# lilijiangg/AutoDiffusion

Hardware: AMD Instinct MI355X
Metric: images/sec (node), ADM-G ImageNet-64 4-step DDIM (higher is better)
Workload: dtype bf16

## Files before the change

autodiffusion_amd/csrc/adm_attention.hip:

```cpp
#include <stdlib.h>

#include <type_traits>

#include "adm_attn_common.h"

namespace {

constexpr int KT = 64;
constexpr int QW = 32;
constexpr int QB = 128;
constexpr int PADE = 16;

#ifdef ADM_ATTN_TIMING
__device__ unsigned long long adm_attn_timing_buf[8 * 65536];
#define ATT_T0() unsigned long long tph[8] = {0, 0, 0, 0, 0, 0, 0, 0}; unsigned long long tlast = __builtin_amdgcn_s_memtime()
#define ATT_T(k) do { const unsigned long long tn_ = __builtin_amdgcn_s_memtime(); tph[k] += tn_ - tlast; tlast = tn_; } while (0)
#define ATT_TEND() do { if (threadIdx.x == 0) { const unsigned b_ = blockIdx.x + gridDim.x * blockIdx.y; if (b_ < 65536) for (int i_ = 0; i_ < 8; ++i_) adm_attn_timing_buf[b_ * 8 + i_] = tph[i_]; } } while (0)
#else
#define ATT_T0() do {} while (0)
#define ATT_T(k) do {} while (0)
#define ATT_TEND() do {} while (0)
#endif

struct AttnK {
  const uint16_t* qkv; uint16_t* out; float* lse;
  const uint16_t* kv;
  int T, heads, C3, C;
  int Tk, kv_rows, Ckv;
  int q_off, k_off, v_off, head_stride, kv_head_stride;
  float scale_log2;
};

template <int D>
__global__ void __launch_bounds__(256, D <= 64 ? 3 : 2)
attn_kernel(const AttnK p) {
  constexpr int KS = D / 32;
  constexpr bool R16 = (D % 32) == 16;
  static_assert(D % 16 == 0 && KS >= 1, "head width must be a multiple of 16, at least 32");
  constexpr int DT = D / 16;
  constexpr float MOVE_THR = 8.0f;
  constexpr bool DMA = D == 64;
  constexpr int KROW = DMA ? D : D + (((D / 2) % 16 == 8) ? 0 : PADE);
  __shared__ __attribute__((aligned(16))) uint16_t Ks[2][KT * KROW];
  __shared__ __attribute__((aligned(16))) uint16_t Vs[2][KT * KROW];

  const int tid = threadIdx.x, lane = tid & 63, wave = tid >> 6;
  const int lc = lane & 15, lq = lane >> 4;
  int bx, by;
  adm_xcd_block(bx, by);
  const int n = by / p.heads, hd = by % p.heads;
  const int qbase = bx * QB + wave * QW;
  const uint16_t* base = p.qkv + (long long)n * p.T * p.C3;
  const int qcol = p.q_off + hd * p.head_stride, kcol = p.k_off + hd * p.kv_head_stride,
            vcol = p.v_off + hd * p.kv_head_stride;
  const __amdgpu_buffer_rsrc_t rsk = __builtin_amdgcn_make_buffer_rsrc((void*)(p.kv + (long long)n * p.kv_rows * p.Ckv), 0,
                                                                       p.Tk * p.Ckv * 2, 0x00020000);

  const __amdgpu_buffer_rsrc_t rs = __builtin_amdgcn_make_buffer_rsrc((void*)base, 0, p.T * p.C3 * 2, 0x00020000);
  adm_h8 qf[2][KS];
#pragma unroll
  for (int qt = 0; qt < 2; ++qt) {
    const int q = qbase + qt * 16 + lc;
#pragma unroll
    for (int ks = 0; ks < KS; ++ks) {
      const adm_u32x4 v = __builtin_amdgcn_raw_buffer_load_b128(rs, (q * p.C3 + qcol + ks * 32 + lq * 8) * 2, 0, 0);
      qf[qt][ks] = __builtin_bit_cast(adm_h8, v);
    }
  }
  adm_s16x4 qf16[2] = {};
  if constexpr (R16) {
#pragma unroll
    for (int qt = 0; qt < 2; ++qt) {
      const int q = qbase + qt * 16 + lc;
      const adm_u32x2 v = __builtin_amdgcn_raw_buffer_load_b64(rs, (q * p.C3 + qcol + KS * 32 + lq * 4) * 2, 0, 0);
      qf16[qt] = __builtin_bit_cast(adm_s16x4, v);
    }
  }

  f32x4 oacc[DT][2], lacc[2], cin[2];
#pragma unroll
  for (int qt = 0; qt < 2; ++qt) {
#pragma unroll
    for (int dt = 0; dt < DT; ++dt) oacc[dt][qt] = f32x4{0.f, 0.f, 0.f, 0.f};
    lacc[qt] = f32x4{0.f, 0.f, 0.f, 0.f};
    cin[qt] = f32x4{0.f, 0.f, 0.f, 0.f};
  }
  float m_run[2] = {0.f, 0.f};
  typedef __attribute__((ext_vector_type(8))) short s16x8;
  const adm_h8 ones = __builtin_bit_cast(adm_h8, s16x8{ADM_ONE16, ADM_ONE16, ADM_ONE16, ADM_ONE16, ADM_ONE16, ADM_ONE16, ADM_ONE16, ADM_ONE16});
  const float thr_raw = MOVE_THR / p.scale_log2;

  const int ntiles = (p.Tk + KT - 1) / KT;
  ATT_T0();
  AdmTileRegs<KT, D, 256> kr, vr;
  typedef __attribute__((ext_vector_type(4))) unsigned int u32x4s;
  const unsigned long long kvbase = (unsigned long long)(p.kv + (long long)n * p.kv_rows * p.Ckv);
  const u32x4s rsk_s = {(unsigned)__builtin_amdgcn_readfirstlane((int)(unsigned)kvbase),
                        (unsigned)__builtin_amdgcn_readfirstlane((int)(unsigned)(kvbase >> 32)) & 0xffffu,
                        (unsigned)__builtin_amdgcn_readfirstlane(p.Tk * p.Ckv * 2), 0x00020000u};
  const unsigned lds_k = (unsigned)(uintptr_t)(__attribute__((address_space(3))) uint16_t*)&Ks[0][0];
  const unsigned lds_v = (unsigned)(uintptr_t)(__attribute__((address_space(3))) uint16_t*)&Vs[0][0];
  const int wave_u = __builtin_amdgcn_readfirstlane(wave);
  auto dma_tile = [&](int kt0) {
    const unsigned slot = (unsigned)(kt0 & 1) * (KT * KROW * 2);
#pragma unroll
    for (int j = 0; j < 2; ++j) {
      const int piece = wave_u * 2 + j;
      const int row = kt0 * KT + piece * 8 + (lane >> 3);
      const int gseg = (lane & 7) ^ (lane >> 3);
      const unsigned voff_k = (unsigned)(row * p.Ckv + kcol + gseg * 8) * 2u, voff_v = (unsigned)(row * p.Ckv + vcol + gseg * 8) * 2u;
      const unsigned dst_k = lds_k + slot + piece * 1024, dst_v = lds_v + slot + piece * 1024;
      unsigned keep;
      asm volatile("s_mov_b32 %0, m0\n\ts_mov_b32 m0, %3\n\ts_nop 0\n\tbuffer_load_dwordx4 %1, %2, 0 offen lds\n\ts_mov_b32 m0, %0"
                   : "=&s"(keep) : "v"(voff_k), "s"(rsk_s), "s"(dst_k) : "memory");
      asm volatile("s_mov_b32 %0, m0\n\ts_mov_b32 m0, %3\n\ts_nop 0\n\tbuffer_load_dwordx4 %1, %2, 0 offen lds\n\ts_mov_b32 m0, %0"
                   : "=&s"(keep) : "v"(voff_v), "s"(rsk_s), "s"(dst_v) : "memory");
    }
  };
  if constexpr (DMA) {
    dma_tile(0);
    asm volatile("s_waitcnt vmcnt(0)" ::: "memory");
  } else {
    kr.load_buf(rsk, p.Ckv, kcol, 0, tid);
    vr.load_buf(rsk, p.Ckv, vcol, 0, tid);
    kr.store(Ks[0], KROW, tid);
    vr.store(Vs[0], KROW, tid);
  }
  __syncthreads();

  auto s_phase = [&](int kt0, f32x4 (&st)[4][2]) {
    const uint16_t* Kc = Ks[kt0 & 1];
    constexpr int NSET = R16 ? 4 : 2;
    adm_h8 kfr[NSET][KS];
    adm_s16x4 kfr16[NSET] = {};
    auto kread = [&](int kt) {
      const int slot = kt % NSET;
#pragma unroll
      for (int ks = 0; ks < KS; ++ks)
        kfr[slot][ks] = *reinterpret_cast<const adm_h8*>(
            &Kc[(kt * 16 + lc) * KROW + (DMA ? ((ks * 4 + lq) ^ (lc & 7)) * 8 : ks * 32 + lq * 8)]);
      if constexpr (R16) kfr16[slot] = *reinterpret_cast<const adm_s16x4*>(&Kc[(kt * 16 + lc) * KROW + KS * 32 + lq * 4]);
    };
    __builtin_amdgcn_sched_barrier(0);
    if constexpr (R16) {
#pragma unroll
      for (int kt = 0; kt < 4; ++kt) kread(kt);
    } else {
      kread(0);
    }
#pragma unroll
    for (int kt = 0; kt < 4; ++kt) {
      if (!R16 && kt + 1 < 4) kread(kt + 1);
      __builtin_amdgcn_sched_barrier(0);
#pragma unroll
      for (int qt = 0; qt < 2; ++qt)
        st[kt][qt] = adm_mfma_16x16x32(kfr[kt % NSET][0], qf[qt][0], cin[qt], 0, 0, 0);
#pragma unroll
      for (int ks = 1; ks < KS; ++ks)
#pragma unroll
        for (int qt = 0; qt < 2; ++qt)
          st[kt][qt] = adm_mfma_16x16x32(kfr[kt % NSET][ks], qf[qt][ks], st[kt][qt], 0, 0, 0);
      if constexpr (R16) {
#pragma unroll
        for (int qt = 0; qt < 2; ++qt)
          st[kt][qt] = adm_mfma_16x16x16(kfr16[kt % NSET], qf16[qt], st[kt][qt], 0, 0, 0);
      }
      __builtin_amdgcn_sched_barrier(0);
    }
  };

  auto tile = [&](int kt0, auto rag_, auto first_) {
    constexpr bool RAG = decltype(rag_)::value, FIRST = decltype(first_)::value;
    const int k0 = kt0 * KT;
    const bool next = kt0 + 1 < ntiles;
    if (next) {
      if constexpr (DMA) {
        dma_tile(kt0 + 1);
      } else {
        kr.load_buf(rsk, p.Ckv, kcol, k0 + KT, tid);
        vr.load_buf(rsk, p.Ckv, vcol, k0 + KT, tid);
      }
    }
    ATT_T(0);
    f32x4 st[4][2];
    s_phase(kt0, st);
    ATT_T(1);
    const uint16_t* Vc = Vs[kt0 & 1];
    __builtin_amdgcn_sched_barrier(0);
    adm_h8 vfr[2][2];
    auto vread = [&](int dt, int slot) {
#pragma unroll
      for (int kb = 0; kb < 2; ++kb)
        vfr[slot][kb] = DMA ? adm_tr_frag_swz(Vc, kb * 32, dt * 16, lc, lq) : adm_tr_frag(Vc, KROW, kb * 32, dt * 16, lc, lq);
    };
    vread(0, 0);
    __builtin_amdgcn_sched_barrier(0);
    ATT_T(2);
    if constexpr (RAG) {
#pragma unroll
// ... 288 lines not shown
```

autodiffusion_amd/csrc/adm_attention_bwd.hip:

```cpp
#include "adm_attn_common.h"

namespace {

constexpr int TT = 64;
constexpr int BW = 32;
constexpr int BB = 128;
constexpr int PADE = 16;

struct AttnBwdK {
  const uint16_t* qkv; const uint16_t* out; const uint16_t* dout; const float* lse; const float* delta;
  float* delta_out;
  uint16_t* dqkv;
  int T, heads, C3, C;
  int q_off, k_off, v_off, head_stride;
  float scale_log2, inv_sqrt_d;
};

template <int D>
__global__ void __launch_bounds__(256, 2)
attn_dq_kernel(const AttnBwdK p) {
  constexpr int KS = D / 32, DT = D / 16, KROW = D + PADE;
  __shared__ __attribute__((aligned(16))) uint16_t Ks[2][TT * KROW];
  __shared__ __attribute__((aligned(16))) uint16_t Vs[2][TT * KROW];
  const int tid = threadIdx.x, lane = tid & 63, wave = tid >> 6, lc = lane & 15, lq = lane >> 4;
  int bx, by;
  adm_xcd_block(bx, by);
  const int n = by / p.heads, hd = by % p.heads;
  const int qbase = bx * BB + wave * BW;
  const uint16_t* base = p.qkv + (long long)n * p.T * p.C3;
  const uint16_t* dbase = p.dout + (long long)n * p.T * p.C;
  const int qcol = p.q_off + hd * p.head_stride, kcol = p.k_off + hd * p.head_stride, vcol = p.v_off + hd * p.head_stride;

  const __amdgpu_buffer_rsrc_t rs = __builtin_amdgcn_make_buffer_rsrc((void*)base, 0, p.T * p.C3 * 2, 0x00020000);
  const __amdgpu_buffer_rsrc_t rsg = __builtin_amdgcn_make_buffer_rsrc((void*)dbase, 0, p.T * p.C * 2, 0x00020000);
  const __amdgpu_buffer_rsrc_t rso = __builtin_amdgcn_make_buffer_rsrc((void*)(p.out + (long long)n * p.T * p.C), 0, p.T * p.C * 2, 0x00020000);
  adm_h8 qf[2][KS], gf[2][KS];
  float lse[2], dl[2];
#pragma unroll
  for (int qt = 0; qt < 2; ++qt) {
    const int q = qbase + qt * 16 + lc;
    const bool ok = q < p.T;
    float dsum = 0.f;
#pragma unroll
    for (int ks = 0; ks < KS; ++ks) {
      const adm_u32x4 a = __builtin_amdgcn_raw_buffer_load_b128(rs, (q * p.C3 + qcol + ks * 32 + lq * 8) * 2, 0, 0);
      const adm_u32x4 g = __builtin_amdgcn_raw_buffer_load_b128(rsg, (q * p.C + hd * D + ks * 32 + lq * 8) * 2, 0, 0);
      const adm_u32x4 o = __builtin_amdgcn_raw_buffer_load_b128(rso, (q * p.C + hd * D + ks * 32 + lq * 8) * 2, 0, 0);
      qf[qt][ks] = __builtin_bit_cast(adm_h8, a);
      gf[qt][ks] = __builtin_bit_cast(adm_h8, g);
#pragma unroll
      for (int e = 0; e < 4; ++e) {
        dsum += adm_lo_f32(o[e]) * adm_lo_f32(g[e]);
        dsum += adm_hi_f32(o[e]) * adm_hi_f32(g[e]);
      }
    }
    dsum = adm_quarter_sum(dsum);
    const long long si = ((long long)n * p.heads + hd) * p.T + (ok ? q : 0);
    lse[qt] = ok ? p.lse[si] : 0.f;
    dl[qt] = dsum;
    if (ok && lq == 0) p.delta_out[si] = dsum;
  }
  f32x4 acc[DT][2];
#pragma unroll
  for (int dt = 0; dt < DT; ++dt)
#pragma unroll
    for (int qt = 0; qt < 2; ++qt) acc[dt][qt] = f32x4{0.f, 0.f, 0.f, 0.f};

  AdmTileRegs<TT, D, 256> kr, vr;
  kr.load_buf(rs, p.C3, kcol, 0, tid);
  vr.load_buf(rs, p.C3, vcol, 0, tid);
  kr.store(Ks[0], KROW, tid);
  vr.store(Vs[0], KROW, tid);
  __syncthreads();

  const int ntiles = (p.T + TT - 1) / TT;
  for (int t0 = 0; t0 < ntiles; ++t0) {
    const int k0 = t0 * TT, cur = t0 & 1;
    const bool next = t0 + 1 < ntiles;
    if (next) {
      kr.load_buf(rs, p.C3, kcol, k0 + TT, tid);
      vr.load_buf(rs, p.C3, vcol, k0 + TT, tid);
    }
    const uint16_t* Kc = Ks[cur];
    const uint16_t* Vc = Vs[cur];
    adm_h8 dsf[2][2];
#pragma unroll
    for (int kb = 0; kb < 2; ++kb) {
      f32x4 st[2][2], dp[2][2];
      const f32x4 zero4 = {0.f, 0.f, 0.f, 0.f};
#pragma unroll
      for (int kk = 0; kk < 2; ++kk) {
        const int kt = 2 * kb + kk;
#pragma unroll
        for (int ks = 0; ks < KS; ++ks) {
          const adm_h8 kf = *reinterpret_cast<const adm_h8*>(&Kc[(kt * 16 + lc) * KROW + ks * 32 + lq * 8]);
          const adm_h8 vf = *reinterpret_cast<const adm_h8*>(&Vc[(kt * 16 + lc) * KROW + ks * 32 + lq * 8]);
#pragma unroll
          for (int qt = 0; qt < 2; ++qt) {
            st[kk][qt] = adm_mfma_16x16x32(kf, qf[qt][ks], ks == 0 ? zero4 : st[kk][qt], 0, 0, 0);
            dp[kk][qt] = adm_mfma_16x16x32(vf, gf[qt][ks], ks == 0 ? zero4 : dp[kk][qt], 0, 0, 0);
          }
        }
      }
#pragma unroll
      for (int qt = 0; qt < 2; ++qt) {
        const adm_f32x2 sc2 = {p.scale_log2, p.scale_log2}, nl2 = {-lse[qt], -lse[qt]}, nd2 = {-dl[qt], -dl[qt]};
        float dsv[8];
#pragma unroll
        for (int kk = 0; kk < 2; ++kk)
#pragma unroll
          for (int h = 0; h < 2; ++h) {
            const adm_f32x2 a = __builtin_elementwise_fma(adm_f32x2{st[kk][qt][2 * h], st[kk][qt][2 * h + 1]}, sc2, nl2);
            const adm_f32x2 pr = {__builtin_amdgcn_exp2f(a.x), __builtin_amdgcn_exp2f(a.y)};
            const adm_f32x2 d2 = pr * (adm_f32x2{dp[kk][qt][2 * h], dp[kk][qt][2 * h + 1]} + nd2);
            dsv[kk * 4 + 2 * h] = d2.x;
            dsv[kk * 4 + 2 * h + 1] = d2.y;
          }
        adm_h8 f;
#pragma unroll
        for (int e = 0; e < 8; ++e) f[e] = (adm_elem_t)dsv[e];
        dsf[qt][kb] = f;
      }
    }
#pragma unroll
    for (int dt = 0; dt < DT; ++dt)
#pragma unroll
      for (int kb = 0; kb < 2; ++kb) {
        const adm_h8 kt_f = adm_tr_frag(Kc, KROW, kb * 32, dt * 16, lc, lq);
#pragma unroll
        for (int qt = 0; qt < 2; ++qt)
          acc[dt][qt] = adm_mfma_16x16x32(kt_f, dsf[qt][kb], acc[dt][qt], 0, 0, 0);
      }
    if (next) {
      kr.store(Ks[cur ^ 1], KROW, tid);
      vr.store(Vs[cur ^ 1], KROW, tid);
    }
    __syncthreads();
  }
#pragma unroll
  for (int qt = 0; qt < 2; ++qt) {
    const int q = qbase + qt * 16 + lc;
    if (q >= p.T) continue;
    uint16_t* orow = p.dqkv + ((long long)n * p.T + q) * p.C3 + qcol;
#pragma unroll
    for (int dt = 0; dt < DT; ++dt) {
      const f32x4 o = acc[dt][qt] * p.inv_sqrt_d;
      uint2 pk;
      pk.x = adm_pack2(o[0], o[1]);
      pk.y = adm_pack2(o[2], o[3]);
      *reinterpret_cast<uint2*>(orow + dt * 16 + lq * 4) = pk;
    }
  }
}

template <int D>
__global__ void __launch_bounds__(256, 2)
attn_dkv_kernel(const AttnBwdK p) {
  constexpr int KS = D / 32, DT = D / 16, KROW = D + PADE;
  __shared__ __attribute__((aligned(16))) uint16_t Qs[2][TT * KROW];
  __shared__ __attribute__((aligned(16))) uint16_t Gs[2][TT * KROW];
  __shared__ __attribute__((aligned(16))) float lse_s[2][TT], dl_s[2][TT];
  const int tid = threadIdx.x, lane = tid & 63, wave = tid >> 6, lc = lane & 15, lq = lane >> 4;
  int bx, by;
  adm_xcd_block(bx, by);
  const int n = by / p.heads, hd = by % p.heads;
  const int kbase = bx * BB + wave * BW;
  const uint16_t* base = p.qkv + (long long)n * p.T * p.C3;
  const uint16_t* dbase = p.dout + (long long)n * p.T * p.C;
  const int qcol = p.q_off + hd * p.head_stride, kcol = p.k_off + hd * p.head_stride, vcol = p.v_off + hd * p.head_stride;
  const long long sbase = ((long long)n * p.heads + hd) * p.T;

  const __amdgpu_buffer_rsrc_t rs = __builtin_amdgcn_make_buffer_rsrc((void*)base, 0, p.T * p.C3 * 2, 0x00020000);
  const __amdgpu_buffer_rsrc_t rsg = __builtin_amdgcn_make_buffer_rsrc((void*)dbase, 0, p.T * p.C * 2, 0x00020000);
  adm_h8 kf[2][KS], vf[2][KS];
#pragma unroll
  for (int kt = 0; kt < 2; ++kt) {
    const int key = kbase + kt * 16 + lc;
#pragma unroll
    for (int ks = 0; ks < KS; ++ks) {
      const adm_u32x4 a = __builtin_amdgcn_raw_buffer_load_b128(rs, (key * p.C3 + kcol + ks * 32 + lq * 8) * 2, 0, 0);
      const adm_u32x4 b = __builtin_amdgcn_raw_buffer_load_b128(rs, (key * p.C3 + vcol + ks * 32 + lq * 8) * 2, 0, 0);
      kf[kt][ks] = __builtin_bit_cast(adm_h8, a);
      vf[kt][ks] = __builtin_bit_cast(adm_h8, b);
    }
  }
  f32x4 dv[DT][2], dk[DT][2];
#pragma unroll
  for (int dt = 0; dt < DT; ++dt)
#pragma unroll
    for (int kt = 0; kt < 2; ++kt) { dv[dt][kt] = f32x4{0.f, 0.f, 0.f, 0.f}; dk[dt][kt] = f32x4{0.f, 0.f, 0.f, 0.f}; }

  AdmTileRegs<TT, D, 256> qr, gr;
  float lse_r = 0.f, dl_r = 0.f;
  auto load_rows = [&](int q0) {
    qr.load_buf(rs, p.C3, qcol, q0, tid);
    gr.load_buf(rsg, p.C, hd * D, q0, tid);
    if (tid < TT) {
      const int q = q0 + tid;
      lse_r = q < p.T ? p.lse[sbase + q] : 1e30f;
      dl_r = q < p.T ? p.delta[sbase + q] : 0.f;
    }
  };
  auto store_rows = [&](int buf) {
    qr.store(Qs[buf], KROW, tid);
    gr.store(Gs[buf], KROW, tid);
    if (tid < TT) { lse_s[buf][tid] = lse_r; dl_s[buf][tid] = dl_r; }
  };
  load_rows(0);
  store_rows(0);
  __syncthreads();

  const int ntiles = (p.T + TT - 1) / TT;
  for (int t0 = 0; t0 < ntiles; ++t0) {
    const int q0 = t0 * TT, cur = t0 & 1;
    const bool next = t0 + 1 < ntiles;
    if (next) load_rows(q0 + TT);
    const uint16_t* Qc = Qs[cur];
    const uint16_t* Gc = Gs[cur];
#pragma unroll
    for (int qb = 0; qb < 2; ++qb) {
      adm_h8 pf[2], dsf[2];
#pragma unroll
      for (int kt = 0; kt < 2; ++kt) {
        f32x4 st[2], dp[2];
        const f32x4 zero4 = {0.f, 0.f, 0.f, 0.f};
#pragma unroll
        for (int qq = 0; qq < 2; ++qq) {
          const int qt = 2 * qb + qq;
#pragma unroll
          for (int ks = 0; ks < KS; ++ks) {
            const adm_h8 qa = *reinterpret_cast<const adm_h8*>(&Qc[(qt * 16 + lc) * KROW + ks * 32 + lq * 8]);
            const adm_h8 ga = *reinterpret_cast<const adm_h8*>(&Gc[(qt * 16 + lc) * KROW + ks * 32 + lq * 8]);
            st[qq] = adm_mfma_16x16x32(qa, kf[kt][ks], ks == 0 ? zero4 : st[qq], 0, 0, 0);
            dp[qq] = adm_mfma_16x16x32(ga, vf[kt][ks], ks == 0 ? zero4 : dp[qq], 0, 0, 0);
          }
        }
        adm_h8 f, g;
        const adm_f32x2 sc2 = {p.scale_log2, p.scale_log2};
#pragma unroll
        for (int qq = 0; qq < 2; ++qq) {
          const int ql = (2 * qb + qq) * 16 + lq * 4;
          const float4 l4 = *reinterpret_cast<const float4*>(&lse_s[cur][ql]);
          const float4 d4 = *reinterpret_cast<const float4*>(&dl_s[cur][ql]);
          const adm_f32x2 a0 = __builtin_elementwise_fma(adm_f32x2{st[qq][0], st[qq][1]}, sc2, adm_f32x2{-l4.x, -l4.y});
          const adm_f32x2 a1 = __builtin_elementwise_fma(adm_f32x2{st[qq][2], st[qq][3]}, sc2, adm_f32x2{-l4.z, -l4.w});
          const adm_f32x2 p0 = {__builtin_amdgcn_exp2f(a0.x), __builtin_amdgcn_exp2f(a0.y)};
          const adm_f32x2 p1 = {__builtin_amdgcn_exp2f(a1.x), __builtin_amdgcn_exp2f(a1.y)};
          const adm_f32x2 s0 = p0 * (adm_f32x2{dp[qq][0], dp[qq][1]} - adm_f32x2{d4.x, d4.y});
          const adm_f32x2 s1 = p1 * (adm_f32x2{dp[qq][2], dp[qq][3]} - adm_f32x2{d4.z, d4.w});
          f[qq * 4 + 0] = (adm_elem_t)p0.x; f[qq * 4 + 1] = (adm_elem_t)p0.y; f[qq * 4 + 2] = (adm_elem_t)p1.x; f[qq * 4 + 3] = (adm_elem_t)p1.y;
          g[qq * 4 + 0] = (adm_elem_t)s0.x; g[qq * 4 + 1] = (adm_elem_t)s0.y; g[qq * 4 + 2] = (adm_elem_t)s1.x; g[qq * 4 + 3] = (adm_elem_t)s1.y;
        }
        pf[kt] = f;
        dsf[kt] = g;
      }
#pragma unroll
      for (int dt = 0; dt < DT; ++dt) {
        const adm_h8 gt_f = adm_tr_frag(Gc, KROW, qb * 32, dt * 16, lc, lq);
        const adm_h8 qt_f = adm_tr_frag(Qc, KROW, qb * 32, dt * 16, lc, lq);
#pragma unroll
        for (int kt = 0; kt < 2; ++kt) {
          dv[dt][kt] = adm_mfma_16x16x32(gt_f, pf[kt], dv[dt][kt], 0, 0, 0);
          dk[dt][kt] = adm_mfma_16x16x32(qt_f, dsf[kt], dk[dt][kt], 0, 0, 0);
        }
      }
    }
    if (next) store_rows(cur ^ 1);
    __syncthreads();
  }
#pragma unroll
  for (int kt = 0; kt < 2; ++kt) {
    const int key = kbase + kt * 16 + lc;
    if (key >= p.T) continue;
    uint16_t* orow = p.dqkv + ((long long)n * p.T + key) * p.C3;
#pragma unroll
    for (int dt = 0; dt < DT; ++dt) {
      const f32x4 a = dk[dt][kt] * p.inv_sqrt_d;
      const f32x4 b = dv[dt][kt];
      uint2 pk;
      pk.x = adm_pack2(a[0], a[1]);
      pk.y = adm_pack2(a[2], a[3]);
      *reinterpret_cast<uint2*>(orow + kcol + dt * 16 + lq * 4) = pk;
      pk.x = adm_pack2(b[0], b[1]);
      pk.y = adm_pack2(b[2], b[3]);
      *reinterpret_cast<uint2*>(orow + vcol + dt * 16 + lq * 4) = pk;
    }
  }
}

}

extern "C" int adm_attention_bwd(const adm_bf16* qkv, const adm_bf16* out, const adm_bf16* dout, const float* lse,
                                 float* delta_ws, adm_bf16* dqkv, int n, int t, int heads, int d, int new_order,
                                 void* stream) {
  ADM_REQUIRE(qkv && out && dout && lse && delta_ws && dqkv, ADM_E_ARG, "adm_attention_bwd: null pointer");
  ADM_REQUIRE(n > 0 && t > 0 && heads > 0, ADM_E_ARG, "adm_attention_bwd: bad shape");
  ADM_REQUIRE(d == 32 || d == 64, ADM_E_SHAPE, "adm_attention_bwd: head dim %d unsupported (32, 64)", d);
  ADM_REQUIRE(adm_aligned16(qkv) && adm_aligned16(out) && adm_aligned16(dout) && adm_aligned16(dqkv), ADM_E_ALIGN,
              "adm_attention_bwd: unaligned pointer");
  ADM_REQUIRE((long long)n * heads < 65536, ADM_E_SHAPE, "adm_attention_bwd: n*heads exceeds grid.y");
  AttnBwdK k{};
  k.qkv = qkv; k.out = out; k.dout = dout; k.lse = lse; k.delta = delta_ws; k.delta_out = delta_ws; k.dqkv = dqkv;
  k.T = t; k.heads = heads; k.C = heads * d; k.C3 = 3 * k.C;
  if (new_order) { k.q_off = 0; k.k_off = k.C; k.v_off = 2 * k.C; k.head_stride = d; }
  else           { k.q_off = 0; k.k_off = d;   k.v_off = 2 * d;   k.head_stride = 3 * d; }
  k.inv_sqrt_d = 1.0f / sqrtf((float)d);
  k.scale_log2 = 1.4426950408889634f * k.inv_sqrt_d;
  hipStream_t s = (hipStream_t)stream;
  dim3 grid((t + BB - 1) / BB, n * heads);
  if (d == 32) {
    hipLaunchKernelGGL((attn_dq_kernel<32>), grid, dim3(256), 0, s, k);
    hipLaunchKernelGGL((attn_dkv_kernel<32>), grid, dim3(256), 0, s, k);
  } else {
    hipLaunchKernelGGL((attn_dq_kernel<64>), grid, dim3(256), 0, s, k);
    hipLaunchKernelGGL((attn_dkv_kernel<64>), grid, dim3(256), 0, s, k);
  }
  return adm_check_launch("adm_attention_bwd");
}
```

autodiffusion_amd/csrc/adm_attn_common.h:

```cpp
#pragma once
#include "adm_common.h"

typedef __attribute__((ext_vector_type(4))) short adm_s16x4;
typedef __attribute__((ext_vector_type(4))) unsigned int adm_u32x4;
typedef __attribute__((ext_vector_type(2))) float adm_f32x2;

__device__ __forceinline__ void adm_xcd_block(int& bx, int& by) {
  const unsigned nx = gridDim.x, total = gridDim.x * gridDim.y;
  const unsigned lin = blockIdx.x + nx * blockIdx.y;
  const unsigned share = total >> 3, rem = total & 7, xcd = lin & 7;
  const unsigned logical = xcd * share + min(xcd, rem) + (lin >> 3);
  bx = (int)(logical % nx);
  by = (int)(logical / nx);
}

__device__ __forceinline__ adm_h8 adm_tr_frag(const uint16_t* tile, int row_stride, int row0, int col0, int lc, int lq) {
  const uint16_t* p0 = tile + (row0 + 4 * lq + (lc >> 2)) * row_stride + col0 + 4 * (lc & 3);
  const adm_s16x4 lo = __builtin_amdgcn_ds_read_tr16_b64_v4i16((__attribute__((address_space(3))) adm_s16x4*)p0);
  const adm_s16x4 hi = __builtin_amdgcn_ds_read_tr16_b64_v4i16(
      (__attribute__((address_space(3))) adm_s16x4*)(p0 + 16 * row_stride));
  typedef __attribute__((ext_vector_type(8))) short s16x8;
  const s16x8 v = {lo[0], lo[1], lo[2], lo[3], hi[0], hi[1], hi[2], hi[3]};
  return __builtin_bit_cast(adm_h8, v);
}

__device__ __forceinline__ adm_h8 adm_tr_frag_swz(const uint16_t* tile, int row0, int col0, int lc, int lq) {
  const int r = 4 * lq + (lc >> 2);
  const int seg = ((col0 >> 3) + ((lc & 3) >> 1)) ^ (r & 7);
  const uint16_t* p0 = tile + (row0 + r) * 64 + seg * 8 + 4 * (lc & 1);
  const adm_s16x4 lo = __builtin_amdgcn_ds_read_tr16_b64_v4i16((__attribute__((address_space(3))) adm_s16x4*)p0);
  const adm_s16x4 hi = __builtin_amdgcn_ds_read_tr16_b64_v4i16((__attribute__((address_space(3))) adm_s16x4*)(p0 + 16 * 64));
  typedef __attribute__((ext_vector_type(8))) short s16x8;
  const s16x8 v = {lo[0], lo[1], lo[2], lo[3], hi[0], hi[1], hi[2], hi[3]};
  return __builtin_bit_cast(adm_h8, v);
}

template <int ROWS, int D, int NT>
struct AdmTileRegs {
  static constexpr int UNITS = ROWS * D / 8;
  static constexpr int PER = (UNITS + NT - 1) / NT;
  uint4 v[PER];
  __device__ __forceinline__ void load(const uint16_t* base, long long row_stride, int col0, int r0, int rmax, int tid) {
#pragma unroll
    for (int i = 0; i < PER; ++i) {
      const int u = tid + i * NT;
      const int r = u / (D / 8), sg = u % (D / 8);
      uint4 x = make_uint4(0, 0, 0, 0);
      if (u < UNITS && r0 + r < rmax) x = *reinterpret_cast<const uint4*>(base + (long long)(r0 + r) * row_stride + col0 + sg * 8);
      v[i] = x;
    }
  }
  __device__ __forceinline__ void load_buf(__amdgpu_buffer_rsrc_t rs, int row_stride, int col0, int r0, int tid) {
#pragma unroll
    for (int i = 0; i < PER; ++i) {
      const int u = tid + i * NT;
      const int r = u / (D / 8), sg = u % (D / 8);
      const unsigned off = u < UNITS ? (unsigned)((r0 + r) * row_stride + col0 + sg * 8) * 2u : 0x80000000u;
      const adm_u32x4 x = __builtin_amdgcn_raw_buffer_load_b128(rs, (int)off, 0, 0);
      v[i] = make_uint4(x[0], x[1], x[2], x[3]);
    }
  }
  __device__ __forceinline__ void store(uint16_t* tile, int krow, int tid) const {
#pragma unroll
    for (int i = 0; i < PER; ++i) {
      const int u = tid + i * NT;
      if (u < UNITS) *reinterpret_cast<uint4*>(&tile[(u / (D / 8)) * krow + (u % (D / 8)) * 8]) = v[i];
    }
  }
};

typedef __attribute__((ext_vector_type(2))) unsigned int adm_u32x2;
__device__ __forceinline__ float adm_quarter_max(float x) {
  adm_u32x2 r = __builtin_amdgcn_permlane16_swap(__float_as_uint(x), __float_as_uint(x), false, false);
  const float m = fmaxf(__uint_as_float(r[0]), __uint_as_float(r[1]));
  r = __builtin_amdgcn_permlane32_swap(__float_as_uint(m), __float_as_uint(m), false, false);
  return fmaxf(__uint_as_float(r[0]), __uint_as_float(r[1]));
}
__device__ __forceinline__ float adm_quarter_sum(float x) {
  adm_u32x2 r = __builtin_amdgcn_permlane16_swap(__float_as_uint(x), __float_as_uint(x), false, false);
  const float m = __uint_as_float(r[0]) + __uint_as_float(r[1]);
  r = __builtin_amdgcn_permlane32_swap(__float_as_uint(m), __float_as_uint(m), false, false);
  return __uint_as_float(r[0]) + __uint_as_float(r[1]);
}
```

Measured before the change: 777.4.

## Use LDS-DMA swizzled tile loads and pipelined fragment reads in attention backward

For head dim 64 and sequence length up to a fixed cap, the dQ and dK/dV attention-backward kernels now stream K/V (or Q/dO) tiles straight into LDS. They use buffer_load...lds DMA into an XOR-swizzled, unpadded layout instead of staging through registers. The inner loops are software-pipelined so the next LDS fragment read is issued while the current MFMAs run, with sched_barriers fencing the phases. The dK/dV kernel preloads all lse/delta values into LDS once, and launch bounds rise to three blocks per CU. The aim is less register pressure and fewer VGPR round trips for tile staging, plus better overlap of LDS reads with MFMA. The cost is a hard sequence-length cap, which also makes the LDS footprint larger, and some shared helpers refactored out of the forward kernel.

```diff
diff --git a/autodiffusion_amd/csrc/adm_attention.hip b/autodiffusion_amd/csrc/adm_attention.hip
--- a/autodiffusion_amd/csrc/adm_attention.hip
+++ b/autodiffusion_amd/csrc/adm_attention.hip
@@ -93,11 +93,7 @@
   const int ntiles = (p.Tk + KT - 1) / KT;
   ATT_T0();
   AdmTileRegs<KT, D, 256> kr, vr;
-  typedef __attribute__((ext_vector_type(4))) unsigned int u32x4s;
-  const unsigned long long kvbase = (unsigned long long)(p.kv + (long long)n * p.kv_rows * p.Ckv);
-  const u32x4s rsk_s = {(unsigned)__builtin_amdgcn_readfirstlane((int)(unsigned)kvbase),
-                        (unsigned)__builtin_amdgcn_readfirstlane((int)(unsigned)(kvbase >> 32)) & 0xffffu,
-                        (unsigned)__builtin_amdgcn_readfirstlane(p.Tk * p.Ckv * 2), 0x00020000u};
+  const adm_rsrc_s rsk_s = adm_dma_rsrc(p.kv + (long long)n * p.kv_rows * p.Ckv, p.Tk, p.Ckv);
   const unsigned lds_k = (unsigned)(uintptr_t)(__attribute__((address_space(3))) uint16_t*)&Ks[0][0];
   const unsigned lds_v = (unsigned)(uintptr_t)(__attribute__((address_space(3))) uint16_t*)&Vs[0][0];
   const int wave_u = __builtin_amdgcn_readfirstlane(wave);
@@ -107,14 +103,11 @@
     for (int j = 0; j < 2; ++j) {
       const int piece = wave_u * 2 + j;
       const int row = kt0 * KT + piece * 8 + (lane >> 3);
-      const int gseg = (lane & 7) ^ (lane >> 3);
+      const int gseg = adm_dma_swz_seg(lane);
       const unsigned voff_k = (unsigned)(row * p.Ckv + kcol + gseg * 8) * 2u, voff_v = (unsigned)(row * p.Ckv + vcol + gseg * 8) * 2u;
       const unsigned dst_k = lds_k + slot + piece * 1024, dst_v = lds_v + slot + piece * 1024;
-      unsigned keep;
-      asm volatile("s_mov_b32 %0, m0\n\ts_mov_b32 m0, %3\n\ts_nop 0\n\tbuffer_load_dwordx4 %1, %2, 0 offen lds\n\ts_mov_b32 m0, %0"
-                   : "=&s"(keep) : "v"(voff_k), "s"(rsk_s), "s"(dst_k) : "memory");
-      asm volatile("s_mov_b32 %0, m0\n\ts_mov_b32 m0, %3\n\ts_nop 0\n\tbuffer_load_dwordx4 %1, %2, 0 offen lds\n\ts_mov_b32 m0, %0"
-                   : "=&s"(keep) : "v"(voff_v), "s"(rsk_s), "s"(dst_v) : "memory");
+      adm_lds_dma_b128(voff_k, rsk_s, dst_k);
+      adm_lds_dma_b128(voff_v, rsk_s, dst_v);
     }
   };
   if constexpr (DMA) {
diff --git a/autodiffusion_amd/csrc/adm_attention_bwd.hip b/autodiffusion_amd/csrc/adm_attention_bwd.hip
--- a/autodiffusion_amd/csrc/adm_attention_bwd.hip
+++ b/autodiffusion_amd/csrc/adm_attention_bwd.hip
@@ -6,6 +6,7 @@
 constexpr int BW = 32;
 constexpr int BB = 128;
 constexpr int PADE = 16;
+constexpr int DMA_MAX_T = 2560;
 
 struct AttnBwdK {
   const uint16_t* qkv; const uint16_t* out; const uint16_t* dout; const float* lse; const float* delta;
@@ -16,10 +17,17 @@
   float scale_log2, inv_sqrt_d;
 };
 
-template <int D>
-__global__ void __launch_bounds__(256, 2)
+__device__ __forceinline__ void adm_landed(adm_h8& x) {
+  adm_u32x4 t = __builtin_bit_cast(adm_u32x4, x);
+  asm volatile("" : "+v"(t));
+  x = __builtin_bit_cast(adm_h8, t);
+}
+
+template <int D, bool DMA>
+__global__ void __launch_bounds__(256, DMA ? 3 : 2)
 attn_dq_kernel(const AttnBwdK p) {
-  constexpr int KS = D / 32, DT = D / 16, KROW = D + PADE;
+  static_assert(!DMA || D == 64, "the LDS-DMA tile layout is 128-byte rows");
+  constexpr int KS = D / 32, DT = D / 16, KROW = DMA ? D : D + PADE;
   __shared__ __attribute__((aligned(16))) uint16_t Ks[2][TT * KROW];
   __shared__ __attribute__((aligned(16))) uint16_t Vs[2][TT * KROW];
   const int tid = threadIdx.x, lane = tid & 63, wave = tid >> 6, lc = lane & 15, lq = lane >> 4;
@@ -66,76 +74,158 @@
 #pragma unroll
     for (int qt = 0; qt < 2; ++qt) acc[dt][qt] = f32x4{0.f, 0.f, 0.f, 0.f};
 
-  AdmTileRegs<TT, D, 256> kr, vr;
-  kr.load_buf(rs, p.C3, kcol, 0, tid);
-  vr.load_buf(rs, p.C3, vcol, 0, tid);
-  kr.store(Ks[0], KROW, tid);
-  vr.store(Vs[0], KROW, tid);
-  __syncthreads();
+  auto ds_frag = [&](const f32x4 (&st)[2][2], const f32x4 (&dp)[2][2], int qt) {
+    const adm_f32x2 sc2 = {p.scale_log2, p.scale_log2}, nl2 = {-lse[qt], -lse[qt]}, nd2 = {-dl[qt], -dl[qt]};
+    float dsv[8];
+#pragma unroll
+    for (int kk = 0; kk < 2; ++kk)
+#pragma unroll
+      for (int h = 0; h < 2; ++h) {
+        const adm_f32x2 a = __builtin_elementwise_fma(adm_f32x2{st[kk][qt][2 * h], st[kk][qt][2 * h + 1]}, sc2, nl2);
+        const adm_f32x2 pr = {__builtin_amdgcn_exp2f(a.x), __builtin_amdgcn_exp2f(a.y)};
+        const adm_f32x2 d2 = pr * (adm_f32x2{dp[kk][qt][2 * h], dp[kk][qt][2 * h + 1]} + nd2);
+        dsv[kk * 4 + 2 * h] = d2.x;
+        dsv[kk * 4 + 2 * h + 1] = d2.y;
+      }
+    adm_h8 f;
+#pragma unroll
+    for (int e = 0; e < 8; ++e) f[e] = (adm_elem_t)dsv[e];
+    return f;
+  };
 
   const int ntiles = (p.T + TT - 1) / TT;
-  for (int t0 = 0; t0 < ntiles; ++t0) {
-    const int k0 = t0 * TT, cur = t0 & 1;
-    const bool next = t0 + 1 < ntiles;
-    if (next) {
-      kr.load_buf(rs, p.C3, kcol, k0 + TT, tid);
-      vr.load_buf(rs, p.C3, vcol, k0 + TT, tid);
-    }
-    const uint16_t* Kc = Ks[cur];
-    const uint16_t* Vc = Vs[cur];
-    adm_h8 dsf[2][2];
-#pragma unroll
-    for (int kb = 0; kb < 2; ++kb) {
-      f32x4 st[2][2], dp[2][2];
-      const f32x4 zero4 = {0.f, 0.f, 0.f, 0.f};
-#pragma unroll
-      for (int kk = 0; kk < 2; ++kk) {
-        const int kt = 2 * kb + kk;
+  if constexpr (DMA) {
+    const adm_rsrc_s rs_s = adm_dma_rsrc(base, p.T, p.C3);
+    const unsigned lds_k = (unsigned)(uintptr_t)(__attribute__((address_space(3))) uint16_t*)&Ks[0][0];
+    const unsigned lds_v = (unsigned)(uintptr_t)(__attribute__((address_space(3))) uint16_t*)&Vs[0][0];
+    const int wave_u = __builtin_amdgcn_readfirstlane(wave);
+    auto dma_tile = [&](int t) {
+      const unsigned slot = (unsigned)(t & 1) * (TT * KROW * 2);
+#pragma unroll
+      for (int j = 0; j < 2; ++j) {
+        const int piece = wave_u * 2 + j;
+        const int row_off = (t * TT + piece * 8 + (lane >> 3)) * p.C3 + adm_dma_swz_seg(lane) * 8;
+        adm_lds_dma_b128((unsigned)(row_off + kcol) * 2u, rs_s, lds_k + slot + piece * 1024);
+        adm_lds_dma_b128((unsigned)(row_off + vcol) * 2u, rs_s, lds_v + slot + piece * 1024);
+      }
+    };
+    dma_tile(0);
+#pragma unroll
+    for (int qt = 0; qt < 2; ++qt)
+#pragma unroll
+      for (int ks = 0; ks < KS; ++ks) { adm_landed(qf[qt][ks]); adm_landed(gf[qt][ks]); }
+    asm volatile("s_waitcnt vmcnt(0)" ::: "memory");
+    __syncthreads();
+    for (int t0 = 0; t0 < ntiles; ++t0) {
+      if (t0 + 1 < ntiles) dma_tile(t0 + 1);
+      const uint16_t* Kc = Ks[t0 & 1];
+      const uint16_t* Vc = Vs[t0 & 1];
+      adm_h8 kfr[2][KS], vfr[2][KS], tfr[2][2];
+      auto sread = [&](int kt) {
 #pragma unroll
         for (int ks = 0; ks < KS; ++ks) {
-          const adm_h8 kf = *reinterpret_cast<const adm_h8*>(&Kc[(kt * 16 + lc) * KROW + ks * 32 + lq * 8]);
-          const adm_h8 vf = *reinterpret_cast<const adm_h8*>(&Vc[(kt * 16 + lc) * KROW + ks * 32 + lq * 8]);
-#pragma unroll
-          for (int qt = 0; qt < 2; ++qt) {
-            st[kk][qt] = adm_mfma_16x16x32(kf, qf[qt][ks], ks == 0 ? zero4 : st[kk][qt], 0, 0, 0);
-            dp[kk][qt] = adm_mfma_16x16x32(vf, gf[qt][ks], ks == 0 ? zero4 : dp[kk][qt], 0, 0, 0);
+          const int off = adm_swz_frag_off(kt * 16 + lc, ks * 4 + lq);
+          kfr[kt & 1][ks] = *reinterpret_cast<const adm_h8*>(&Kc[off]);
+          vfr[kt & 1][ks] = *reinterpret_cast<const adm_h8*>(&Vc[off]);
+        }
+      };
+      auto tread = [&](int dt) {
+#pragma unroll
+        for (int kb = 0; kb < 2; ++kb) tfr[dt & 1][kb] = adm_tr_frag_swz(Kc, kb * 32, dt * 16, lc, lq);
+      };
+      adm_h8 dsf[2][2];
+      __builtin_amdgcn_sched_barrier(0);
+      sread(0);
+#pragma unroll
+      for (int kb = 0; kb < 2; ++kb) {
+        f32x4 st[2][2], dp[2][2];
+        const f32x4 zero4 = {0.f, 0.f, 0.f, 0.f};
+#pragma unroll
+        for (int kk = 0; kk < 2; ++kk) {
+          const int kt = 2 * kb + kk;
+          if (kt + 1 < 4) sread(kt + 1); else tread(0);
+          __builtin_amdgcn_sched_barrier(0);
+#pragma unroll
+          for (int ks = 0; ks < KS; ++ks)
+#pragma unroll
+            for (int qt = 0; qt < 2; ++qt) {
+              st[kk][qt] = adm_mfma_16x16x32(kfr[kt & 1][ks], qf[qt][ks], ks == 0 ? zero4 : st[kk][qt], 0, 0, 0);
+              dp[kk][qt] = adm_mfma_16x16x32(vfr[kt & 1][ks], gf[qt][ks], ks == 0 ? zero4 : dp[kk][qt], 0, 0, 0);
+            }
+          __builtin_amdgcn_sched_barrier(0);
+        }
+#pragma unroll
+        for (int qt = 0; qt < 2; ++qt) dsf[qt][kb] = ds_frag(st, dp, qt);
+      }
+      __builtin_amdgcn_sched_barrier(0);
+#pragma unroll
+      for (int dt = 0; dt < DT; ++dt) {
+        if (dt + 1 < DT) tread(dt + 1);
+        __builtin_amdgcn_sched_barrier(0);
+#pragma unroll
+        for (int kb = 0; kb < 2; ++kb)
+#pragma unroll
+          for (int qt = 0; qt < 2; ++qt)
+            acc[dt][qt] = adm_mfma_16x16x32(tfr[dt & 1][kb], dsf[qt][kb], acc[dt][qt], 0, 0, 0);
+        __builtin_amdgcn_sched_barrier(0);
+      }
+      asm volatile("s_waitcnt vmcnt(0)" ::: "memory");
+      __syncthreads();
+    }
+  } else {
+    AdmTileRegs<TT, D, 256> kr, vr;
+    kr.load_buf(rs, p.C3, kcol, 0, tid);
+    vr.load_buf(rs, p.C3, vcol, 0, tid);
+    kr.store(Ks[0], KROW, tid);
+    vr.store(Vs[0], KROW, tid);
+    __syncthreads();
+
+    for (int t0 = 0; t0 < ntiles; ++t0) {
+      const int k0 = t0 * TT, cur = t0 & 1;
+      const bool next = t0 + 1 < ntiles;
+      if (next) {
+        kr.load_buf(rs, p.C3, kcol, k0 + TT, tid);
+        vr.load_buf(rs, p.C3, vcol, k0 + TT, tid);
+      }
+      const uint16_t* Kc = Ks[cur];
+      const uint16_t* Vc = Vs[cur];
+      adm_h8 dsf[2][2];
+#pragma unroll
+      for (int kb = 0; kb < 2; ++kb) {
+        f32x4 st[2][2], dp[2][2];
+        const f32x4 zero4 = {0.f, 0.f, 0.f, 0.f};
+#pragma unroll
+        for (int kk = 0; kk < 2; ++kk) {
+          const int kt = 2 * kb + kk;
+#pragma unroll
+          for (int ks = 0; ks < KS; ++ks) {
+            const adm_h8 kf = *reinterpret_cast<const adm_h8*>(&Kc[(kt * 16 + lc) * KROW + ks * 32 + lq * 8]);
+            const adm_h8 vf = *reinterpret_cast<const adm_h8*>(&Vc[(kt * 16 + lc) * KROW + ks * 32 + lq * 8]);
+#pragma unroll
+            for (int qt = 0; qt < 2; ++qt) {
+              st[kk][qt] = adm_mfma_16x16x32(kf, qf[qt][ks], ks == 0 ? zero4 : st[kk][qt], 0, 0, 0);
+              dp[kk][qt] = adm_mfma_16x16x32(vf, gf[qt][ks], ks == 0 ? zero4 : dp[kk][qt], 0, 0, 0);
+            }
           }
         }
-      }
-#pragma unroll
-      for (int qt = 0; qt < 2; ++qt) {
-        const adm_f32x2 sc2 = {p.scale_log2, p.scale_log2}, nl2 = {-lse[qt], -lse[qt]}, nd2 = {-dl[qt], -dl[qt]};
-        float dsv[8];
-#pragma unroll
-        for (int kk = 0; kk < 2; ++kk)
-#pragma unroll
-          for (int h = 0; h < 2; ++h) {
-            const adm_f32x2 a = __builtin_elementwise_fma(adm_f32x2{st[kk][qt][2 * h], st[kk][qt][2 * h + 1]}, sc2, nl2);
-            const adm_f32x2 pr = {__builtin_amdgcn_exp2f(a.x), __builtin_amdgcn_exp2f(a.y)};
-            const adm_f32x2 d2 = pr * (adm_f32x2{dp[kk][qt][2 * h], dp[kk][qt][2 * h + 1]} + nd2);
-            dsv[kk * 4 + 2 * h] = d2.x;
-            dsv[kk * 4 + 2 * h + 1] = d2.y;
-          }
-        adm_h8 f;
-#pragma unroll
-        for (int e = 0; e < 8; ++e) f[e] = (adm_elem_t)dsv[e];
-        dsf[qt][kb] = f;
-      }
-    }
-#pragma unroll
-    for (int dt = 0; dt < DT; ++dt)
-#pragma unroll
-      for (int kb = 0; kb < 2; ++kb) {
-        const adm_h8 kt_f = adm_tr_frag(Kc, KROW, kb * 32, dt * 16, lc, lq);
-#pragma unroll
-        for (int qt = 0; qt < 2; ++qt)
-          acc[dt][qt] = adm_mfma_16x16x32(kt_f, dsf[qt][kb], acc[dt][qt], 0, 0, 0);
-      }
-    if (next) {
-      kr.store(Ks[cur ^ 1], KROW, tid);
-      vr.store(Vs[cur ^ 1], KROW, tid);
-    }
-    __syncthreads();
+#pragma unroll
+        for (int qt = 0; qt < 2; ++qt) dsf[qt][kb] = ds_frag(st, dp, qt);
+      }
+#pragma unroll
+      for (int dt = 0; dt < DT; ++dt)
+#pragma unroll
+        for (int kb = 0; kb < 2; ++kb) {
+          const adm_h8 kt_f = adm_tr_frag(Kc, KROW, kb * 32, dt * 16, lc, lq);
+#pragma unroll
+          for (int qt = 0; qt < 2; ++qt)
+            acc[dt][qt] = adm_mfma_16x16x32(kt_f, dsf[qt][kb], acc[dt][qt], 0, 0, 0);
+        }
+      if (next) {
+        kr.store(Ks[cur ^ 1], KROW, tid);
+        vr.store(Vs[cur ^ 1], KROW, tid);
+      }
+      __syncthreads();
+    }
   }
 #pragma unroll
   for (int qt = 0; qt < 2; ++qt) {
@@ -153,13 +243,13 @@
   }
 }
 
-template <int D>
-__global__ void __launch_bounds__(256, 2)
+template <int D, bool DMA>
+__global__ void __launch_bounds__(256, DMA ? 3 : 2)
 attn_dkv_kernel(const AttnBwdK p) {
-  constexpr int KS = D / 32, DT = D / 16, KROW = D + PADE;
+  static_assert(!DMA || D == 64, "the LDS-DMA tile layout is 128-byte rows");
+  constexpr int KS = D / 32, DT = D / 16, KROW = DMA ? D : D + PADE;
   __shared__ __attribute__((aligned(16))) uint16_t Qs[2][TT * KROW];
   __shared__ __attribute__((aligned(16))) uint16_t Gs[2][TT * KROW];
-  __shared__ __attribute__((aligned(16))) float lse_s[2][TT], dl_s[2][TT];
   const int tid = threadIdx.x, lane = tid & 63, wave = tid >> 6, lc = lane & 15, lq = lane >> 4;
   int bx, by;
   adm_xcd_block(bx, by);
@@ -190,83 +280,166 @@
 #pragma unroll
     for (int kt = 0; kt < 2; ++kt) { dv[dt][kt] = f32x4{0.f, 0.f, 0.f, 0.f}; dk[dt][kt] = f32x4{0.f, 0.f, 0.f, 0.f}; }
 
-  AdmTileRegs<TT, D, 256> qr, gr;
-  float lse_r = 0.f, dl_r = 0.f;
-  auto load_rows = [&](int q0) {
-    qr.load_buf(rs, p.C3, qcol, q0, tid);
-    gr.load_buf(rsg, p.C, hd * D, q0, tid);
-    if (tid < TT) {
-      const int q = q0 + tid;
-      lse_r = q < p.T ? p.lse[sbase + q] : 1e30f;
-      dl_r = q < p.T ? p.delta[sbase + q] : 0.f;
-    }
+  auto p_ds_frags = [&](const f32x4 (&st)[2], const f32x4 (&dp)[2], const float* l, const float* d, adm_h8& pf, adm_h8& dsf) {
+    adm_h8 f, g;
+    const adm_f32x2 sc2 = {p.scale_log2, p.scale_log2};
+#pragma unroll
+    for (int qq = 0; qq < 2; ++qq) {
+      const float4 l4 = *reinterpret_cast<const float4*>(l + qq * 16);
+      const float4 d4 = *reinterpret_cast<const float4*>(d + qq * 16);
+      const adm_f32x2 a0 = __builtin_elementwise_fma(adm_f32x2{st[qq][0], st[qq][1]}, sc2, adm_f32x2{-l4.x, -l4.y});
+      const adm_f32x2 a1 = __builtin_elementwise_fma(adm_f32x2{st[qq][2], st[qq][3]}, sc2, adm_f32x2{-l4.z, -l4.w});
+      const adm_f32x2 p0 = {__builtin_amdgcn_exp2f(a0.x), __builtin_amdgcn_exp2f(a0.y)};
+      const adm_f32x2 p1 = {__builtin_amdgcn_exp2f(a1.x), __builtin_amdgcn_exp2f(a1.y)};
+      const adm_f32x2 s0 = p0 * (adm_f32x2{dp[qq][0], dp[qq][1]} - adm_f32x2{d4.x, d4.y});
+      const adm_f32x2 s1 = p1 * (adm_f32x2{dp[qq][2], dp[qq][3]} - adm_f32x2{d4.z, d4.w});
+      f[qq * 4 + 0] = (adm_elem_t)p0.x; f[qq * 4 + 1] = (adm_elem_t)p0.y; f[qq * 4 + 2] = (adm_elem_t)p1.x; f[qq * 4 + 3] = (adm_elem_t)p1.y;
+      g[qq * 4 + 0] = (adm_elem_t)s0.x; g[qq * 4 + 1] = (adm_elem_t)s0.y; g[qq * 4 + 2] = (adm_elem_t)s1.x; g[qq * 4 + 3] = (adm_elem_t)s1.y;
+    }
+    pf = f;
+    dsf = g;
   };
-  auto store_rows = [&](int buf) {
-    qr.store(Qs[buf], KROW, tid);
-    gr.store(Gs[buf], KROW, tid);
-    if (tid < TT) { lse_s[buf][tid] = lse_r; dl_s[buf][tid] = dl_r; }
-  };
-  load_rows(0);
-  store_rows(0);
-  __syncthreads();
 
   const int ntiles = (p.T + TT - 1) / TT;
-  for (int t0 = 0; t0 < ntiles; ++t0) {
-    const int q0 = t0 * TT, cur = t0 & 1;
-    const bool next = t0 + 1 < ntiles;
-    if (next) load_rows(q0 + TT);
-    const uint16_t* Qc = Qs[cur];
-    const uint16_t* Gc = Gs[cur];
-#pragma unroll
-    for (int qb = 0; qb < 2; ++qb) {
-      adm_h8 pf[2], dsf[2];
-#pragma unroll
-      for (int kt = 0; kt < 2; ++kt) {
-        f32x4 st[2], dp[2];
-        const f32x4 zero4 = {0.f, 0.f, 0.f, 0.f};
-#pragma unroll
-        for (int qq = 0; qq < 2; ++qq) {
-          const int qt = 2 * qb + qq;
-#pragma unroll
-          for (int ks = 0; ks < KS; ++ks) {
-            const adm_h8 qa = *reinterpret_cast<const adm_h8*>(&Qc[(qt * 16 + lc) * KROW + ks * 32 + lq * 8]);
-            const adm_h8 ga = *reinterpret_cast<const adm_h8*>(&Gc[(qt * 16 + lc) * KROW + ks * 32 + lq * 8]);
-            st[qq] = adm_mfma_16x16x32(qa, kf[kt][ks], ks == 0 ? zero4 : st[qq], 0, 0, 0);
-            dp[qq] = adm_mfma_16x16x32(ga, vf[kt][ks], ks == 0 ? zero4 : dp[qq], 0, 0, 0);
+  if constexpr (DMA) {
+    __shared__ __attribute__((aligned(16))) float lse_s[DMA_MAX_T], dl_s[DMA_MAX_T];
+    for (int q = tid; q < ntiles * TT; q += 256) {
+      lse_s[q] = q < p.T ? p.lse[sbase + q] : 1e30f;
+      dl_s[q] = q < p.T ? p.delta[sbase + q] : 0.f;
+    }
+    const adm_rsrc_s rs_s = adm_dma_rsrc(base, p.T, p.C3), rsg_s = adm_dma_rsrc(dbase, p.T, p.C);
+    const unsigned lds_q = (unsigned)(uintptr_t)(__attribute__((address_space(3))) uint16_t*)&Qs[0][0];
+    const unsigned lds_g = (unsigned)(uintptr_t)(__attribute__((address_space(3))) uint16_t*)&Gs[0][0];
+    const int wave_u = __builtin_amdgcn_readfirstlane(wave);
+    auto dma_tile = [&](int t) {
+      const unsigned slot = (unsigned)(t & 1) * (TT * KROW * 2);
+#pragma unroll
+      for (int j = 0; j < 2; ++j) {
+        const int piece = wave_u * 2 + j;
+        const int row = t * TT + piece * 8 + (lane >> 3), gseg = adm_dma_swz_seg(lane);
+        adm_lds_dma_b128((unsigned)(row * p.C3 + qcol + gseg * 8) * 2u, rs_s, lds_q + slot + piece * 1024);
+        adm_lds_dma_b128((unsigned)(row * p.C + hd * D + gseg * 8) * 2u, rsg_s, lds_g + slot + piece * 1024);
+      }
+    };
+    dma_tile(0);
+#pragma unroll
+    for (int kt = 0; kt < 2; ++kt)
+#pragma unroll
+      for (int ks = 0; ks < KS; ++ks) { adm_landed(kf[kt][ks]); adm_landed(vf[kt][ks]); }
+    asm volatile("s_waitcnt vmcnt(0)" ::: "memory");
+    __syncthreads();
+    for (int t0 = 0; t0 < ntiles; ++t0) {
+      if (t0 + 1 < ntiles) dma_tile(t0 + 1);
+      const uint16_t* Qc = Qs[t0 & 1];
+      const uint16_t* Gc = Gs[t0 & 1];
+      adm_h8 qfr[2], gfr[2], tqr[2], tgr[2];
+      auto sread = [&](int qb, int i) {
+        const int off = adm_swz_frag_off((2 * qb + (i & 1)) * 16 + lc, (i >> 1) * 4 + lq);
+        qfr[i & 1] = *reinterpret_cast<const adm_h8*>(&Qc[off]);
+        gfr[i & 1] = *reinterpret_cast<const adm_h8*>(&Gc[off]);
+      };
+      auto tread = [&](int qb, int dt) {
+        tgr[dt & 1] = adm_tr_frag_swz(Gc, qb * 32, dt * 16, lc, lq);
+        tqr[dt & 1] = adm_tr_frag_swz(Qc, qb * 32, dt * 16, lc, lq);
+      };
+      __builtin_amdgcn_sched_barrier(0);
+      sread(0, 0);
+#pragma unroll
+      for (int qb = 0; qb < 2; ++qb) {
+        adm_h8 pf[2], dsf[2];
+#pragma unroll
+        for (int kt = 0; kt < 2; ++kt) {
+          f32x4 st[2], dp[2];
+          const f32x4 zero4 = {0.f, 0.f, 0.f, 0.f};
+#pragma unroll
+          for (int i = 0; i < 4; ++i) {
+            const int qq = i & 1, ks = i >> 1;
+            if (i + 1 < 4) sread(qb, i + 1); else if (kt == 0) sread(qb, 0); else tread(qb, 0);
+            __builtin_amdgcn_sched_barrier(0);
+            st[qq] = adm_mfma_16x16x32(qfr[i & 1], kf[kt][ks], ks == 0 ? zero4 : st[qq], 0, 0, 0);
+            dp[qq] = adm_mfma_16x16x32(gfr[i & 1], vf[kt][ks], ks == 0 ? zero4 : dp[qq], 0, 0, 0);
+            __builtin_amdgcn_sched_barrier(0);
           }
-        }
-        adm_h8 f, g;
-        const adm_f32x2 sc2 = {p.scale_log2, p.scale_log2};
-#pragma unroll
-        for (int qq = 0; qq < 2; ++qq) {
-          const int ql = (2 * qb + qq) * 16 + lq * 4;
-          const float4 l4 = *reinterpret_cast<const float4*>(&lse_s[cur][ql]);
-          const float4 d4 = *reinterpret_cast<const float4*>(&dl_s[cur][ql]);
-          const adm_f32x2 a0 = __builtin_elementwise_fma(adm_f32x2{st[qq][0], st[qq][1]}, sc2, adm_f32x2{-l4.x, -l4.y});
-          const adm_f32x2 a1 = __builtin_elementwise_fma(adm_f32x2{st[qq][2], st[qq][3]}, sc2, adm_f32x2{-l4.z, -l4.w});
-          const adm_f32x2 p0 = {__builtin_amdgcn_exp2f(a0.x), __builtin_amdgcn_exp2f(a0.y)};
-          const adm_f32x2 p1 = {__builtin_amdgcn_exp2f(a1.x), __builtin_amdgcn_exp2f(a1.y)};
-          const adm_f32x2 s0 = p0 * (adm_f32x2{dp[qq][0], dp[qq][1]} - adm_f32x2{d4.x, d4.y});
-          const adm_f32x2 s1 = p1 * (adm_f32x2{dp[qq][2], dp[qq][3]} - adm_f32x2{d4.z, d4.w});
-          f[qq * 4 + 0] = (adm_elem_t)p0.x; f[qq * 4 + 1] = (adm_elem_t)p0.y; f[qq * 4 + 2] = (adm_elem_t)p1.x; f[qq * 4 + 3] = (adm_elem_t)p1.y;
-          g[qq * 4 + 0] = (adm_elem_t)s0.x; g[qq * 4 + 1] = (adm_elem_t)s0.y; g[qq * 4 + 2] = (adm_elem_t)s1.x; g[qq * 4 + 3] = (adm_elem_t)s1.y;
-        }
-        pf[kt] = f;
-        dsf[kt] = g;
-      }
-#pragma unroll
-      for (int dt = 0; dt < DT; ++dt) {
-        const adm_h8 gt_f = adm_tr_frag(Gc, KROW, qb * 32, dt * 16, lc, lq);
-        const adm_h8 qt_f = adm_tr_frag(Qc, KROW, qb * 32, dt * 16, lc, lq);
+          p_ds_frags(st, dp, &lse_s[t0 * TT + qb * 32 + lq * 4], &dl_s[t0 * TT + qb * 32 + lq * 4], pf[kt], dsf[kt]);
+        }
+        __builtin_amdgcn_sched_barrier(0);
+#pragma unroll
+        for (int dt = 0; dt < DT; ++dt) {
+          if (dt + 1 < DT) tread(qb, dt + 1); else if (qb == 0) sread(1, 0);
+          __builtin_amdgcn_sched_barrier(0);
+#pragma unroll
+          for (int kt = 0; kt < 2; ++kt) {
+            dv[dt][kt] = adm_mfma_16x16x32(tgr[dt & 1], pf[kt], dv[dt][kt], 0, 0, 0);
+            dk[dt][kt] = adm_mfma_16x16x32(tqr[dt & 1], dsf[kt], dk[dt][kt], 0, 0, 0);
+          }
+          __builtin_amdgcn_sched_barrier(0);
+        }
+      }
+      asm volatile("s_waitcnt vmcnt(0)" ::: "memory");
+      __syncthreads();
+    }
+  } else {
+    __shared__ __attribute__((aligned(16))) float lse_s[2][TT], dl_s[2][TT];
+    AdmTileRegs<TT, D, 256> qr, gr;
+    float lse_r = 0.f, dl_r = 0.f;
+    auto load_rows = [&](int q0) {
+      qr.load_buf(rs, p.C3, qcol, q0, tid);
+      gr.load_buf(rsg, p.C, hd * D, q0, tid);
+      if (tid < TT) {
+        const int q = q0 + tid;
+        lse_r = q < p.T ? p.lse[sbase + q] : 1e30f;
+        dl_r = q < p.T ? p.delta[sbase + q] : 0.f;
+      }
+    };
+    auto store_rows = [&](int buf) {
+      qr.store(Qs[buf], KROW, tid);
+      gr.store(Gs[buf], KROW, tid);
+      if (tid < TT) { lse_s[buf][tid] = lse_r; dl_s[buf][tid] = dl_r; }
+    };
+    load_rows(0);
+    store_rows(0);
+    __syncthreads();
+
+    for (int t0 = 0; t0 < ntiles; ++t0) {
+      const int q0 = t0 * TT, cur = t0 & 1;
+      const bool next = t0 + 1 < ntiles;
+      if (next) load_rows(q0 + TT);
+      const uint16_t* Qc = Qs[cur];
+      const uint16_t* Gc = Gs[cur];
+#pragma unroll
+      for (int qb = 0; qb < 2; ++qb) {
+        adm_h8 pf[2], dsf[2];
 #pragma unroll
         for (int kt = 0; kt < 2; ++kt) {
-          dv[dt][kt] = adm_mfma_16x16x32(gt_f, pf[kt], dv[dt][kt], 0, 0, 0);
-          dk[dt][kt] = adm_mfma_16x16x32(qt_f, dsf[kt], dk[dt][kt], 0, 0, 0);
-        }
-      }
-    }
-    if (next) store_rows(cur ^ 1);
-    __syncthreads();
+          f32x4 st[2], dp[2];
+          const f32x4 zero4 = {0.f, 0.f, 0.f, 0.f};
+#pragma unroll
+          for (int qq = 0; qq < 2; ++qq) {
+            const int qt = 2 * qb + qq;
+#pragma unroll
+            for (int ks = 0; ks < KS; ++ks) {
+              const adm_h8 qa = *reinterpret_cast<const adm_h8*>(&Qc[(qt * 16 + lc) * KROW + ks * 32 + lq * 8]);
+              const adm_h8 ga = *reinterpret_cast<const adm_h8*>(&Gc[(qt * 16 + lc) * KROW + ks * 32 + lq * 8]);
+              st[qq] = adm_mfma_16x16x32(qa, kf[kt][ks], ks == 0 ? zero4 : st[qq], 0, 0, 0);
+              dp[qq] = adm_mfma_16x16x32(ga, vf[kt][ks], ks == 0 ? zero4 : dp[qq], 0, 0, 0);
+            }
+          }
+          p_ds_frags(st, dp, &lse_s[cur][qb * 32 + lq * 4], &dl_s[cur][qb * 32 + lq * 4], pf[kt], dsf[kt]);
+        }
+#pragma unroll
+        for (int dt = 0; dt < DT; ++dt) {
+          const adm_h8 gt_f = adm_tr_frag(Gc, KROW, qb * 32, dt * 16, lc, lq);
+          const adm_h8 qt_f = adm_tr_frag(Qc, KROW, qb * 32, dt * 16, lc, lq);
+#pragma unroll
+          for (int kt = 0; kt < 2; ++kt) {
+            dv[dt][kt] = adm_mfma_16x16x32(gt_f, pf[kt], dv[dt][kt], 0, 0, 0);
+            dk[dt][kt] = adm_mfma_16x16x32(qt_f, dsf[kt], dk[dt][kt], 0, 0, 0);
+          }
+        }
+      }
+      if (next) store_rows(cur ^ 1);
+      __syncthreads();
+    }
   }
 #pragma unroll
   for (int kt = 0; kt < 2; ++kt) {
@@ -309,11 +482,14 @@
   hipStream_t s = (hipStream_t)stream;
   dim3 grid((t + BB - 1) / BB, n * heads);
   if (d == 32) {
-    hipLaunchKernelGGL((attn_dq_kernel<32>), grid, dim3(256), 0, s, k);
-    hipLaunchKernelGGL((attn_dkv_kernel<32>), grid, dim3(256), 0, s, k);
+    hipLaunchKernelGGL((attn_dq_kernel<32, false>), grid, dim3(256), 0, s, k);
+    hipLaunchKernelGGL((attn_dkv_kernel<32, false>), grid, dim3(256), 0, s, k);
+  } else if (t <= DMA_MAX_T) {
+    hipLaunchKernelGGL((attn_dq_kernel<64, true>), grid, dim3(256), 0, s, k);
+    hipLaunchKernelGGL((attn_dkv_kernel<64, true>), grid, dim3(256), 0, s, k);
   } else {
-    hipLaunchKernelGGL((attn_dq_kernel<64>), grid, dim3(256), 0, s, k);
-    hipLaunchKernelGGL((attn_dkv_kernel<64>), grid, dim3(256), 0, s, k);
+    hipLaunchKernelGGL((attn_dq_kernel<64, false>), grid, dim3(256), 0, s, k);
+    hipLaunchKernelGGL((attn_dkv_kernel<64, false>), grid, dim3(256), 0, s, k);
   }
   return adm_check_launch("adm_attention_bwd");
 }
diff --git a/autodiffusion_amd/csrc/adm_attn_common.h b/autodiffusion_amd/csrc/adm_attn_common.h
--- a/autodiffusion_amd/csrc/adm_attn_common.h
+++ b/autodiffusion_amd/csrc/adm_attn_common.h
@@ -34,6 +34,21 @@
   const s16x8 v = {lo[0], lo[1], lo[2], lo[3], hi[0], hi[1], hi[2], hi[3]};
   return __builtin_bit_cast(adm_h8, v);
 }
+
+typedef __attribute__((ext_vector_type(4))) unsigned int adm_rsrc_s;
+__device__ __forceinline__ adm_rsrc_s adm_dma_rsrc(const void* base, int rows, int pitch) {
+  const unsigned long long b = (unsigned long long)base;
+  return adm_rsrc_s{(unsigned)__builtin_amdgcn_readfirstlane((int)(unsigned)b),
+                    (unsigned)__builtin_amdgcn_readfirstlane((int)(unsigned)(b >> 32)) & 0xffffu,
+                    (unsigned)__builtin_amdgcn_readfirstlane(rows * pitch * 2), 0x00020000u};
+}
+__device__ __forceinline__ void adm_lds_dma_b128(unsigned voff, adm_rsrc_s rs, unsigned lds_dst) {
+  unsigned keep;
+  asm volatile("s_mov_b32 %0, m0\n\ts_mov_b32 m0, %3\n\ts_nop 0\n\tbuffer_load_dwordx4 %1, %2, 0 offen lds\n\ts_mov_b32 m0, %0"
+               : "=&s"(keep) : "v"(voff), "s"(rs), "s"(lds_dst) : "memory");
+}
+__device__ __forceinline__ int adm_dma_swz_seg(int lane) { return (lane & 7) ^ (lane >> 3); }
+__device__ __forceinline__ int adm_swz_frag_off(int row, int seg) { return row * 64 + ((seg ^ (row & 7)) * 8); }
 
 template <int ROWS, int D, int NT>
 struct AdmTileRegs {
```

Result: no change. 783.9 (median of 4 runs) (+0.8%).
